# sp-uhh/audio-visual-vad

Measured on NVIDIA B200. Metric: AV-VAD frames/sec (device-timed), higher is better.
Workload: dtype bf16

## Files before the change

### audio-visual-vad_b200/avvad/lib.py

```python
from __future__ import annotations

import ctypes as C
import os
from typing import Optional

_HERE = os.path.dirname(os.path.abspath(__file__))
LIB_PATH = os.path.join(os.path.dirname(_HERE), "lib", "libavvad.so")

c_i32p = C.POINTER(C.c_int32)
c_i64p = C.POINTER(C.c_int64)
c_f32p = C.POINTER(C.c_float)
VP = C.c_void_p

PROTOTYPES = {
    "avvad_last_error": (C.c_char_p, []),
    "avvad_version": (C.c_int, []),
    "avvad_launch_count": (C.c_uint64, []),
    "avvad_profile_enable": (C.c_int, [C.c_int]),
    "avvad_profile_read": (C.c_int, [C.c_int, C.POINTER(C.c_double), C.POINTER(C.c_double), C.POINTER(C.c_uint64)]),
    "avvad_profile_clear": (C.c_int, []),
    "avvad_profile_dump": (C.c_int64, [C.c_int, C.POINTER(C.c_double), C.POINTER(C.c_double), C.c_int64]),
    "avvad_debug_lstm_trace": (None, [VP]),
    "avvad_stft_num_frames": (C.c_int64, [C.c_int64, C.c_double, C.c_double, C.c_double, C.c_int]),
    "avvad_frontend_logpower": (C.c_int, [VP, C.c_int64, VP, VP, C.c_int32, C.c_int32, C.c_int, VP, VP, C.c_float,
                                          VP, VP, VP]),
    "avvad_stft": (C.c_int, [VP, C.c_int64, VP, VP, C.c_int32, C.c_int32, VP, VP]),
    "avvad_upsampled_length": (C.c_int64, [C.c_int64, C.c_int32, C.c_int32]),
    "avvad_upsample_gather": (C.c_int, [VP, C.c_int, VP, VP, C.c_int32, C.c_int32, C.c_int32, C.c_int32, C.c_int32,
                                        C.c_int32, C.c_float, C.c_float, C.c_float, C.c_int, VP, VP]),
    "avvad_upsample_index": (C.c_int, [C.c_int32, C.c_int32, C.c_int32, C.c_int32, VP, VP]),
    "avvad_resnet18_create": (C.c_int, [C.POINTER(VP)]),
    "avvad_resnet18_destroy": (None, [VP]),
    "avvad_resnet18_set_conv": (C.c_int, [VP, C.c_int, VP, VP, VP, VP, VP, C.c_float, VP]),
    "avvad_resnet18_workspace_bytes": (C.c_size_t, [C.c_int64, C.c_int64]),
    "avvad_resnet18_forward": (C.c_int, [VP, VP, C.c_int64, C.c_int64, VP, C.c_size_t, VP, VP, C.c_int64, C.c_int64,
                                         VP]),
    "avvad_resnet18_forward_u8": (C.c_int, [VP, VP, VP, VP, C.c_int32, C.c_int32, C.c_int32, C.c_int32, C.c_int32,
                                            C.c_float, C.c_float, C.c_float, C.c_int, C.c_int64, VP, C.c_size_t, VP, VP,
                                            C.c_int64, C.c_int64, VP]),
    "avvad_resnet18_forward_upto": (C.c_int, [VP, VP, C.c_int64, C.c_int, VP, C.c_size_t, VP, VP]),
    "avvad_resnet18_set_conv_train": (C.c_int, [VP, C.c_int, VP, VP, VP, VP]),
    "avvad_resnet18_train_workspace_bytes": (C.c_size_t, [C.c_int64]),
    "avvad_resnet18_forward_train": (C.c_int, [VP, VP, C.c_int64, VP, C.c_size_t, C.c_float, C.c_float, VP, VP, VP, VP,
                                               C.c_int64, C.c_int64, VP]),
    "avvad_resnet18_tape_bytes": (C.c_size_t, [C.c_int64]),
    "avvad_resnet18_tape_workspace_bytes": (C.c_size_t, [C.c_int64]),
    "avvad_resnet18_tape_layout": (C.c_int, [C.c_int64, c_i64p, C.c_int]),
    "avvad_resnet18_forward_tape": (C.c_int, [VP, VP, C.c_int64, VP, C.c_size_t, VP, C.c_size_t, C.c_float, C.c_float, VP,
                                              VP, VP, VP, C.c_int64, C.c_int64, VP]),
    "avvad_resnet18_backward_workspace_bytes": (C.c_size_t, [C.c_int64]),
    "avvad_resnet18_backward": (C.c_int, [VP, VP, C.c_int64, VP, VP, VP, C.c_size_t, C.c_float, VP, VP, VP, VP]),
    "avvad_gemm_bf16": (C.c_int, [VP, C.c_int64, VP, C.c_int64, VP, VP, C.c_int64, C.c_int, C.c_int, C.c_int64,
                                  C.c_int64, C.c_int64, VP]),
    "avvad_conv2d_nhwc_bf16": (C.c_int, [VP, VP, VP, VP, VP, C.c_int64, C.c_int, C.c_int, C.c_int, C.c_int, C.c_int,
                                         C.c_int, C.c_int, C.c_int, C.c_int, VP]),
    "avvad_dct_roi_workspace_bytes": (C.c_size_t, [C.c_int64]),
    "avvad_dct_roi_decode": (C.c_int, [VP, C.c_int64, C.c_int, VP, VP, VP, C.c_size_t, VP]),
    "avvad_vad_labels": (C.c_int, [VP, C.c_int64, VP, VP, C.c_int32, C.c_int32, C.c_int32, C.c_int32, C.c_double, VP, VP,
                                   VP]),
    "avvad_ibm_labels": (C.c_int, [VP, VP, C.c_int32, C.c_int32, C.c_int32, C.c_float, C.c_float, VP, VP, VP, VP]),
    "avvad_stats_accumulate": (C.c_int, [VP, VP, C.c_int32, C.c_int32, C.c_int32, VP, VP, VP]),
    "avvad_stats_finalize": (C.c_int, [VP, VP, C.c_double, C.c_int32, VP, VP, VP]),
    "avvad_feature_gather": (C.c_int, [VP, VP, VP, VP, C.c_int32, C.c_int32, C.c_int32, C.c_int32, C.c_int32, C.c_int32,
                                       VP, VP, C.c_int64, C.c_int64, VP]),
    "avvad_conv2d_nhwc_bf16_dual": (C.c_int, [VP, VP, VP, VP, VP, C.c_int64] + [C.c_int] * 13 + [VP]),
    "avvad_pack_rows_bf16": (C.c_int, [VP, C.c_int64, VP, C.c_int64, C.c_int64, C.c_int64, C.c_int64, C.c_int, VP]),
    "avvad_mcb_create": (C.c_int, [C.POINTER(VP)]),
    "avvad_mcb_destroy": (None, [VP]),
    "avvad_mcb_load": (C.c_int, [VP, VP, VP, VP, VP, VP, VP, VP, VP, C.c_float, VP]),
    "avvad_mcb_workspace_bytes": (C.c_size_t, [C.c_int64]),
    "avvad_mcb_forward": (C.c_int, [VP, VP, VP, C.c_int64, VP, C.c_size_t, VP, C.c_int64, VP, VP]),
    "avvad_mcb_grouped_workspace_bytes": (C.c_size_t, [C.c_int64, C.c_int64]),
# ... 84 lines not shown
```

### audio-visual-vad_b200/csrc/resnet.cu

```cuda
#include <stdlib.h>

#include <mutex>

#include "gemm_tma.cuh"
#include "stem_s2d.cuh"

namespace avvad {
namespace tc {
int launch_block17(const __nv_bfloat16* x, const __nv_bfloat16* wa, const float* bias_a, const __nv_bfloat16* wb,
                   const float* bias_b, __nv_bfloat16* z, int64_t n, cudaStream_t st);
bool block17_enabled();
}
}

namespace avvad {

struct ConvSpec {
  int cin, cout, k, stride, pad, hin, hout;
};
static const ConvSpec kSpecs[20] = {
    {3, 64, 7, 2, 3, 67, 34},
    {64, 64, 3, 1, 1, 17, 17},   {64, 64, 3, 1, 1, 17, 17},
    {64, 64, 3, 1, 1, 17, 17},   {64, 64, 3, 1, 1, 17, 17},
    {64, 128, 3, 2, 1, 17, 9},   {128, 128, 3, 1, 1, 9, 9},  {64, 128, 1, 2, 0, 17, 9},
// ... 349 lines not shown
  if (chunk <= 0) chunk = 2048;
  return n_frames < chunk ? n_frames : chunk;
}

extern "C" size_t avvad_resnet18_workspace_bytes(int64_t n_frames, int64_t chunk_frames) {
  if (n_frames <= 0) return 0;
  const int64_t mc = chunk_of(n_frames, chunk_frames);
  return (size_t)(4 * align_up((size_t)mc * kActBytesPerFrame, 1024));
}

static int run_conv(avvad_resnet18* h, int layer, const __nv_bfloat16* in, const __nv_bfloat16* residual,
                    __nv_bfloat16* out, int64_t n, int relu, cudaStream_t st) {
  const ConvSpec& s = kSpecs[layer];
  return avvad_conv2d_nhwc_bf16(in, h->w[layer], h->bias[layer], residual, out, n, s.hin, s.hin, s.cin, s.cout, s.k,
                                s.k, s.stride, s.pad, relu, st);
}

struct StemInput {
  const float* frames = nullptr;
  const uint8_t* src = nullptr;
  const int32_t* n_src = nullptr;
  const int32_t* n_out = nullptr;
  int f_max = 0, t_max = 0, num = 0, den = 0, standardise = 0;
  int64_t src_bytes = 0;
  float mean = 0.f, denom = 1.f;
  StemInput advance(int64_t f0) const {
    StemInput r = *this;
    r.first = first + f0;
    return r;
  }
  int64_t first = 0;
};

static int launch_stem_s2d(avvad_resnet18* h, const StemInput& in, int64_t n, __nv_bfloat16* out, cudaStream_t st,
                           const __nv_bfloat16* w = nullptr, const float* bias = nullptr, double* stats = nullptr) {
  static PerDeviceOnce once;
  AVVAD_CUDA(once.run([] {
    cudaError_t e = cudaFuncSetAttribute(tc::stem_s2d_kernel<0>, cudaFuncAttributeMaxDynamicSharedMemorySize, (int)tc::kS2Smem);
    if (e == cudaSuccess)
      e = cudaFuncSetAttribute(tc::stem_s2d_kernel<1>, cudaFuncAttributeMaxDynamicSharedMemorySize, (int)tc::kS2Smem);
    if (e == cudaSuccess)
      e = cudaFuncSetAttribute(tc::stem_s2d_kernel<0, true>, cudaFuncAttributeMaxDynamicSharedMemorySize, (int)tc::kS2Smem);
    return e;
  }));
  static int num_sms = [] {
    int dev = 0, v = 148;
    if (cudaGetDevice(&dev) == cudaSuccess) cudaDeviceGetAttribute(&v, cudaDevAttrMultiProcessorCount, dev);
    return v > 0 ? v : 148;
  }();
  tc::StemS2Params p{};
  p.n_frames = n;
  p.w1b = w ? w : h->w1b;
  p.bias = w ? bias : h->bias[0];
  p.out = out;
  p.stats = stats;
  const int64_t batches = (n + tc::kS2FramesPerBatch - 1) / tc::kS2FramesPerBatch;
  const unsigned grid = (unsigned)(batches < num_sms ? batches : num_sms);
  void* tok = nullptr;
  tc::prof_begin(st, &tok);
  if (in.src) {
    p.src = in.src; p.n_src = in.n_src; p.n_out = in.n_out; p.src_bytes = in.src_bytes;
    p.f_max = in.f_max; p.t_max = in.t_max; p.num = in.num; p.den = in.den;
    p.mean = in.mean; p.denom = in.denom; p.standardise = in.standardise;
    p.first = in.first;
    tc::stem_s2d_kernel<1><<<grid, tc::kS2Threads, tc::kS2Smem, st>>>(p);
  } else if (stats) {
    p.frames = in.frames + in.first * kFrameHW;
    tc::stem_s2d_kernel<0, true><<<grid, tc::kS2Threads, tc::kS2Smem, st>>>(p);
  } else {
    p.frames = in.frames + in.first * kFrameHW;
    tc::stem_s2d_kernel<0><<<grid, tc::kS2Threads, tc::kS2Smem, st>>>(p);
  }
  AVVAD_LAUNCHED();
  tc::prof_end(st, tok, 3, 2.0 * (double)n * 1156 * 64 * 49);
  return AVVAD_OK;
}

static int launch_stem(avvad_resnet18* h, const StemInput& in, int64_t n, __nv_bfloat16* out, cudaStream_t st) {
  return launch_stem_s2d(h, in, n, out, st);
}

static const int64_t kStageIn[4] = {17 * 17 * 64, 17 * 17 * 64, 9 * 9 * 128, 5 * 5 * 256};
static const int64_t kStageOut[4] = {17 * 17 * 64, 9 * 9 * 128, 5 * 5 * 256, 3 * 3 * 512};
static const double kStageMac[4] = {42614784.0, 42467328.0, 52428800.0, 75497472.0};

static int run_trunk_chunk(avvad_resnet18* h, const StemInput& in, int64_t n, __nv_bfloat16* const buf[4], int upto,
                           int* last, cudaStream_t st) {
  if (fuse_ds()) {
    int frc = build_fused(h, st);
    if (frc) return frc;
  }
  const bool whole = upto < 20;
  int cur = 0;
  *last = cur;
  int layer = 1;
  for (int stage = 0; stage < 4; ++stage) {
    {
      const int64_t f0 = 0, nn = n;
// ... 102 lines not shown
        buf[last], n, 9, 512, feat ? feat + f0 * 512 : nullptr,
        feat_bf16 ? (__nv_bfloat16*)feat_bf16 + f0 * ld_bf16 : nullptr, ld_bf16, col_off);
    AVVAD_LAUNCHED();
  }
  return AVVAD_OK;
}

extern "C" int avvad_resnet18_forward(avvad_resnet18* h, const float* frames, int64_t n_frames, int64_t chunk_frames,
                                      void* workspace, size_t workspace_bytes, float* feat, void* feat_bf16,
                                      int64_t ld_bf16, int64_t col_off, void* stream) {
  AVVAD_CHECK_ARG(h && frames && workspace && n_frames > 0, "bad argument");
  StemInput in;
  in.frames = frames;
  return forward_common(h, in, n_frames, chunk_frames, workspace, workspace_bytes, feat, feat_bf16, ld_bf16, col_off,
                        (cudaStream_t)stream);
}

extern "C" int avvad_resnet18_forward_u8(avvad_resnet18* h, const uint8_t* src, const int32_t* n_src,
                                         const int32_t* n_out, int32_t B, int32_t f_max, int32_t t_max, int32_t num,
                                         int32_t den, float mean, float stdv, float eps, int standardise,
                                         int64_t chunk_frames, void* workspace, size_t workspace_bytes, float* feat,
                                         void* feat_bf16, int64_t ld_bf16, int64_t col_off, void* stream) {
  AVVAD_CHECK_ARG(h && src && n_src && n_out && workspace, "null pointer");
  AVVAD_CHECK_ARG(B > 0 && f_max > 0 && t_max > 0 && num > 0 && den > 0, "non-positive size");
  StemInput in;
  in.src = src; in.n_src = n_src; in.n_out = n_out;
  in.f_max = f_max; in.t_max = t_max; in.num = num; in.den = den;
  in.mean = mean; in.denom = stdv + eps; in.standardise = standardise;
  in.src_bytes = (int64_t)B * f_max * kFrameHW;
  return forward_common(h, in, (int64_t)B * t_max, chunk_frames, workspace, workspace_bytes, feat, feat_bf16, ld_bf16,
                        col_off, (cudaStream_t)stream);
}

extern "C" int avvad_resnet18_forward_upto(avvad_resnet18* h, const float* frames, int64_t n_frames, int upto,
                                           void* workspace, size_t workspace_bytes, void* out_act, void* stream) {
  AVVAD_CHECK_ARG(h && frames && workspace && out_act && n_frames > 0 && upto >= 0 && upto < 20, "bad argument");
  int rc = check_loaded(h);
  if (rc) return rc;
  if (workspace_bytes < avvad_resnet18_workspace_bytes(n_frames, n_frames)) {
    set_error("resnet18: workspace too small (forward_upto runs a single chunk)");
    return AVVAD_ERR_WORKSPACE;
  }
  cudaStream_t st = (cudaStream_t)stream;
  const size_t bsz = align_up((size_t)n_frames * kActBytesPerFrame, 1024);
  __nv_bfloat16* buf[4];
  for (int i = 0; i < 4; ++i) buf[i] = reinterpret_cast<__nv_bfloat16*>((uint8_t*)workspace + i * bsz);
  int last = 0;
  StemInput in;
  in.frames = frames;
  rc = run_trunk_chunk(h, in, n_frames, buf, upto, &last, st);
  if (rc) return rc;
  const ConvSpec& s = kSpecs[upto];
  const int ho = (upto == 0) ? 17 : s.hout;
  const size_t bytes = (size_t)n_frames * ho * ho * s.cout * sizeof(__nv_bfloat16);
  AVVAD_CUDA(cudaMemcpyAsync(out_act, buf[last], bytes, cudaMemcpyDeviceToDevice, st));
  return AVVAD_OK;
}

extern "C" int avvad_resnet18_set_conv_train(avvad_resnet18* h, int layer, const float* w, const float* gamma,
                                             const float* beta, void* stream) {
  AVVAD_CHECK_ARG(h && layer >= 0 && layer < 20 && w && gamma && beta, "bad argument");
  cudaStream_t st = (cudaStream_t)stream;
  const ConvSpec& s = kSpecs[layer];
  const size_t wn = (layer == 0) ? 64 * 64 : (size_t)s.cout * s.cin * s.k * s.k;
  if (!h->wraw[layer]) {
    AVVAD_CUDA(cudaMalloc(&h->wraw[layer], wn * sizeof(__nv_bfloat16)));
// ... 142 lines not shown
```

### audio-visual-vad_b200/csrc/stem_s2d.cuh

```cuda
#pragma once
#include "gemm_tc.cuh"

namespace avvad {
namespace tc {

constexpr int kS2Builders = 256;
constexpr int kS2BuilderWarps = kS2Builders / 32;
constexpr int kS2EpiWarps = 8;
constexpr int kS2EpiThreads = kS2EpiWarps * 32;
constexpr int kS2ChPerWarp = 64 / (kS2EpiWarps / 4);
constexpr int kS2Passes = kS2ChPerWarp / 16;
constexpr int kS2Items = (67 * 37 + kS2Builders - 1) / kS2Builders;
constexpr int kS2Threads = kS2Builders + 32 + kS2EpiThreads;
constexpr int kS2FramesPerBatch = 2;
constexpr int kS2RowsPerFrame = 37;
constexpr int kS2Pitch = 160;
constexpr int kS2PlaneRows = 83;
constexpr uint32_t kS2PlaneBytes = kS2PlaneRows * kS2Pitch;
constexpr int kS2EdgeRows = 132;
constexpr uint32_t kS2EdgeChunkBytes = kS2EdgeRows * 16;
constexpr uint32_t kS2EdgePlaneBytes = 2 * kS2EdgeChunkBytes;
constexpr uint32_t kS2BufBytes = 2 * kS2PlaneBytes + 2 * kS2EdgePlaneBytes;
constexpr uint32_t kS2WStepBytes = 256 * 32;
constexpr uint32_t kS2WBytes = 8 * kS2WStepBytes;
constexpr uint32_t kS2OnesBytes = 128 * 32;
constexpr int kS2RingRows = 32;
constexpr uint32_t kS2RingRowBytes = 16 * 128;
constexpr uint32_t kS2RingBytes = kS2RingRows * kS2RingRowBytes;
constexpr uint32_t kS2EdgeHpBytes = 80 * 128;
constexpr uint32_t kS2OffW = 2 * kS2BufBytes;
constexpr uint32_t kS2OffOnes = kS2OffW + kS2WBytes;
constexpr uint32_t kS2OffRing = kS2OffOnes + kS2OnesBytes;
constexpr uint32_t kS2OffEdgeHp = kS2OffRing + kS2RingBytes;
constexpr uint32_t kS2OffLut = kS2OffEdgeHp + kS2EdgeHpBytes;
constexpr uint32_t kS2OffBias = kS2OffLut + 512;
constexpr uint32_t kS2OffBar = kS2OffBias + 256;
constexpr uint32_t kS2StageBytes = 288 * 16;
constexpr uint32_t kS2OffStage = kS2OffBar + 128;
constexpr uint32_t kS2Smem = 1024 + kS2OffStage + 2 * kS2StageBytes;
static_assert(kS2Smem <= 227 * 1024, "stem kernel: shared memory");

struct StemS2Params {
  const float* frames;
  const uint8_t* src;
  const int32_t* n_src;
  const int32_t* n_out;
  int f_max, t_max, num, den;
  float mean, denom;
  int standardise;
  int64_t n_frames;
  int64_t first;
  const __nv_bfloat16* w1b;
  int64_t src_bytes;
  const float* bias;
  __nv_bfloat16* out;
  double* stats;
};

__device__ __forceinline__ uint32_t desc_lo_ns(uint32_t saddr, uint32_t lbo_bytes) {
  return ((saddr & 0x3FFFFu) >> 4) | ((lbo_bytes >> 4) << 16);
}
__device__ __forceinline__ uint32_t desc_hi_ns(uint32_t sbo_bytes) { return (sbo_bytes >> 4) | (1u << 14); }

__device__ __forceinline__ void umma_f16_ns(uint32_t tmem_d, uint32_t a_lo, uint32_t a_hi, uint32_t b_lo, uint32_t b_hi,
                                            uint32_t idesc, uint32_t accum) {
  asm volatile(
      "{\n\t.reg .pred p;\n\t.reg .b64 da, db;\n\t"
      "mov.b64 da, {%1, %2};\n\t"
      "mov.b64 db, {%3, %4};\n\t"
      "setp.ne.b32 p, %6, 0;\n\t"
      "tcgen05.mma.cta_group::1.kind::f16 [%0], da, db, %5, p;\n\t}"
      ::"r"(tmem_d), "r"(a_lo), "r"(a_hi), "r"(b_lo), "r"(b_hi), "r"(idesc), "r"(accum)
      : "memory");
}

__device__ __forceinline__ int s2_src_index(int k, int n_src, int num, int den) {
  long long v = ((long long)den * (2LL * k + 1) - 1) / (2LL * num);
  return v < n_src - 1 ? (int)v : n_src - 1;
}

__device__ __forceinline__ void named_bar_sync(int id, int nthreads) {
  asm volatile("bar.sync %0, %1;" ::"r"(id), "r"(nthreads) : "memory");
}

__device__ __forceinline__ uint32_t bf16x2_max(uint32_t a, uint32_t b) {
  uint32_t r;
  asm("max.bf16x2 %0, %1, %2;" : "=r"(r) : "r"(a), "r"(b));
  return r;
}

template <int MODE, bool STATS = false>
__global__ void __launch_bounds__(kS2Threads, 1) stem_s2d_kernel(const StemS2Params p) {
  extern __shared__ uint8_t smem_raw[];
  const uint32_t raw = smem_u32(smem_raw);
  const uint32_t base = (raw + 1023u) & ~1023u;
  uint8_t* smem = smem_raw + (base - raw);
  float* bias_s = reinterpret_cast<float*>(smem + kS2OffBias);
  unsigned short* lut = reinterpret_cast<unsigned short*>(smem + kS2OffLut);
  const uint32_t bar0 = base + kS2OffBar;
  auto BAR = [&](int i) { return bar0 + 8u * (uint32_t)i; };
  volatile uint32_t* tmem_slot = reinterpret_cast<volatile uint32_t*>(smem + kS2OffBar + 96);

  const int tid = threadIdx.x;
  const int warp = tid >> 5, lane = tid & 31;
  const int64_t n_batches = (p.n_frames + kS2FramesPerBatch - 1) / kS2FramesPerBatch;

  for (uint32_t i = tid; i < (2 * kS2BufBytes) / 16; i += kS2Threads)
    reinterpret_cast<uint4*>(smem)[i] = make_uint4(0u, 0u, 0u, 0u);
  for (int idx = tid; idx < 7 * 256 * 16; idx += kS2Threads) {
    const int e = idx & 15, n = (idx >> 4) & 255, fr = idx >> 12;
    const int s = n >> 6, ch = n & 63;
    const int fs = e - 2 * s;
    __nv_bfloat16 v = __float2bfloat16_rn(0.f);
    if (fs >= 0 && fs < 7) v = p.w1b[ch * 64 + fr * 7 + fs];
    const uint32_t off = kS2OffW + (uint32_t)fr * kS2WStepBytes + (uint32_t)(n >> 3) * 256u + (uint32_t)(e >> 3) * 128u +
                         (uint32_t)(n & 7) * 16u + (uint32_t)(e & 7) * 2u;
    *reinterpret_cast<__nv_bfloat16*>(smem + off) = v;
  }
  for (int idx = tid; idx < 256 * 16; idx += kS2Threads) {
    const int e = idx & 15, n = idx >> 4;
    const float bv = p.bias ? p.bias[n & 63] : 0.f;
    const __nv_bfloat16 hi = __float2bfloat16_rn(bv);
    __nv_bfloat16 v = __float2bfloat16_rn(0.f);
    if (e == 0) v = hi;
    if (e == 1) v = __float2bfloat16_rn(bv - __bfloat162float(hi));
    const uint32_t off = kS2OffW + 7u * kS2WStepBytes + (uint32_t)(n >> 3) * 256u + (uint32_t)(e >> 3) * 128u +
                         (uint32_t)(n & 7) * 16u + (uint32_t)(e & 7) * 2u;
    *reinterpret_cast<__nv_bfloat16*>(smem + off) = v;
  }
  for (uint32_t i = tid; i < kS2OnesBytes / 4; i += kS2Threads)
    reinterpret_cast<uint32_t*>(smem + kS2OffOnes)[i] = 0x3F803F80u;
  if (tid < 64) bias_s[tid] = p.bias ? p.bias[tid] : 0.f;
  if (MODE == 1 && tid < 256) {
    float v = (float)tid;
    if (p.standardise) v = (v - p.mean) / p.denom;
    const __nv_bfloat16 h = __float2bfloat16_rn(v);
    lut[tid] = *reinterpret_cast<const unsigned short*>(&h);
  }
// ... 101 lines not shown
    fetch((int64_t)blockIdx.x * kS2FramesPerBatch);
    for (int64_t bi = blockIdx.x; bi < n_batches; bi += gridDim.x, ++it) {
      const uint32_t buf = it & 1u;
      mbar_wait(BAR(2 + buf), ((it >> 1) & 1u) ^ 1u);
      uint8_t* bufp = smem + buf * kS2BufBytes;
#pragma unroll
      for (int fi = 0; fi < kS2FramesPerBatch; ++fi) {
        const int64_t n = bi * kS2FramesPerBatch + fi;
        const bool have = n < p.n_frames;
        if (have) store();
        if (MODE == 0 && have) build(bufp, fi);
        const int64_t nn = (fi + 1 < kS2FramesPerBatch) ? n + 1 : (bi + gridDim.x) * kS2FramesPerBatch;
        if (fi + 1 < kS2FramesPerBatch || bi + gridDim.x < n_batches) fetch(nn);
        if (MODE == 1 && have) {
          named_bar_sync(2, kS2Builders);
          build(bufp, fi);
        }
      }
      fence_proxy_async();
      mbar_arrive(BAR(0 + buf));
    }
  } else if (warp == kS2BuilderWarps) {
    constexpr uint32_t idesc = make_idesc(256);
    const uint32_t a_hi_main = desc_hi_ns(kS2Pitch), a_hi_edge = desc_hi_ns(128), b_hi = desc_hi_ns(256);
    uint32_t it = 0, g = 0;
    for (int64_t bi = blockIdx.x; bi < n_batches; bi += gridDim.x, ++it) {
      const uint32_t buf = it & 1u;
      const int nf = (int)((p.n_frames - bi * kS2FramesPerBatch) < kS2FramesPerBatch
                               ? (p.n_frames - bi * kS2FramesPerBatch)
                               : kS2FramesPerBatch);
      const int n_main = (nf * kS2RowsPerFrame + 15) / 16;
      mbar_wait(BAR(0 + buf), (it >> 1) & 1u);
      tc_fence_after();
      const uint32_t bufa = base + buf * kS2BufBytes;
      for (int t = -1; t < n_main; ++t, ++g) {
        const uint32_t acc = g & 1u;
        mbar_wait(BAR(6 + acc), ((g >> 1) & 1u) ^ 1u);
        tc_fence_after();
        if (elect_one_sync()) {
          const uint32_t d = tmem_acc + acc * 256u;
          umma_f16_ns(d, desc_lo_ns(base + kS2OffOnes, 128u), b_hi, desc_lo_ns(base + kS2OffW + 7u * kS2WStepBytes, 128u),
                      b_hi, idesc, 0);
#pragma unroll
          for (int fr = 0; fr < 7; ++fr) {
            const int a = fr >> 1, b = fr & 1;
            uint32_t a_lo, a_hi;
            if (t < 0) {
              a_lo = desc_lo_ns(bufa + 2 * kS2PlaneBytes + (uint32_t)b * kS2EdgePlaneBytes + (uint32_t)a * 16u,
                                kS2EdgeChunkBytes);
              a_hi = a_hi_edge;
            } else {
              a_lo = desc_lo_ns(bufa + (uint32_t)b * kS2PlaneBytes + (uint32_t)(16 * t + a) * kS2Pitch, 16u);
              a_hi = a_hi_main;
            }
            const uint32_t b_lo = desc_lo_ns(base + kS2OffW + (uint32_t)fr * kS2WStepBytes, 128u);
            umma_f16_ns(d, a_lo, a_hi, b_lo, b_hi, idesc, 1);
          }
          umma_commit(BAR(4 + acc));
          if (t == n_main - 1) umma_commit(BAR(2 + buf));
        }
        __syncwarp();
      }
    }
  } else {
    const int ew = warp - (kS2BuilderWarps + 1);
    const int q = warp & 3;
    const int half = ew >> 2;
    const int etid = tid - (kS2Builders + 32);
    const int L = q * 32 + lane;
    uint8_t* ring = smem + kS2OffRing;
    uint8_t* edge_hp = smem + kS2OffEdgeHp;
    uint32_t g = 0;
    if (STATS) {
      float sa[kS2ChPerWarp], sq[kS2ChPerWarp];
#pragma unroll
      for (int c = 0; c < kS2ChPerWarp; ++c) sa[c] = sq[c] = 0.f;
      for (int64_t bi = blockIdx.x; bi < n_batches; bi += gridDim.x) {
        const int nf = (int)((p.n_frames - bi * kS2FramesPerBatch) < kS2FramesPerBatch
                                 ? (p.n_frames - bi * kS2FramesPerBatch)
                                 : kS2FramesPerBatch);
        const int n_rows = nf * kS2RowsPerFrame;
        const int n_main = (n_rows + 15) / 16;
        for (int t = -1; t < n_main; ++t, ++g) {
          const uint32_t acc = g & 1u;
          mbar_wait(BAR(4 + acc), (g >> 1) & 1u);
          tc_fence_after();
          const uint32_t t_row = tmem_acc + acc * 256u + ((uint32_t)(q * 32) << 16);
          const int yy = (t < 0) ? L : 16 * t + (L >> 3);
          const int y = yy % kS2RowsPerFrame;
          const bool live = (yy < n_rows) && (y < 34) && (t >= 0 || L < 80);
          const int s_first = (t < 0) ? 2 : 0;
#pragma unroll 1
          for (int pass = 0; pass < kS2Passes; ++pass) {
            const int ch0 = half * kS2ChPerWarp + pass * 16;
#pragma unroll
            for (int sft = 0; sft < 4; ++sft) {
              uint32_t v[16];
              tmem_ld16(t_row + (uint32_t)sft * 64u + ch0, v);
              tmem_ld_wait();
              if (live && sft >= s_first) {
#pragma unroll
                for (int c = 0; c < 16; ++c) {
                  const float x = __uint_as_float(v[c]);
                  if (kS2Passes == 1 || pass == 0) {
                    sa[c] += x;
// ... 5 lines not shown
                }
              }
            }
          }
          tc_fence_before();
          __syncwarp();
          if (lane == 0) mbar_arrive(BAR(6 + acc));
        }
      }
#pragma unroll
      for (int c = 0; c < kS2ChPerWarp; ++c) {
        float a = sa[c], b = sq[c];
#pragma unroll
        for (int o = 16; o > 0; o >>= 1) {
          a += __shfl_xor_sync(0xffffffffu, a, o);
          b += __shfl_xor_sync(0xffffffffu, b, o);
        }
        if (lane == 0) {
          atomicAdd(p.stats + half * kS2ChPerWarp + c, (double)a);
          atomicAdd(p.stats + 64 + half * kS2ChPerWarp + c, (double)b);
        }
      }
    } else
    for (int64_t bi = blockIdx.x; bi < n_batches; bi += gridDim.x) {
      const int nf = (int)((p.n_frames - bi * kS2FramesPerBatch) < kS2FramesPerBatch
                               ? (p.n_frames - bi * kS2FramesPerBatch)
                               : kS2FramesPerBatch);
      const int n_rows = nf * kS2RowsPerFrame;
      const int n_main = (n_rows + 15) / 16;
      for (int t = -1; t < n_main; ++t, ++g) {
        const uint32_t acc = g & 1u;
        mbar_wait(BAR(4 + acc), (g >> 1) & 1u);
        tc_fence_after();
        const uint32_t t_row = tmem_acc + acc * 256u + ((uint32_t)(q * 32) << 16);
        if (t < 0) {
#pragma unroll 1
          for (int pass = 0; pass < kS2Passes; ++pass) {
            const int ch0 = half * kS2ChPerWarp + pass * 16;
            uint32_t v1[16], v2[16], v3[16];
            tmem_ld16(t_row + 64u + ch0, v1);
            tmem_ld16(t_row + 128u + ch0, v2);
            tmem_ld16(t_row + 192u + ch0, v3);
            tmem_ld_wait();
            if (L < 80) {
              uint32_t o[8];
#pragma unroll
              for (int c = 0; c < 8; ++c) {
                const float x0 = fmaxf(fmaxf(__uint_as_float(v1[2 * c]), __uint_as_float(v2[2 * c])), __uint_as_float(v3[2 * c]));
                const float x1 = fmaxf(fmaxf(__uint_as_float(v1[2 * c + 1]), __uint_as_float(v2[2 * c + 1])),
                                       __uint_as_float(v3[2 * c + 1]));
                o[c] = pack_relu_bf16x2(x0, x1);
              }
              uint8_t* rowp = edge_hp + L * 128;
              const int k0 = ch0 >> 3;
              *reinterpret_cast<uint4*>(rowp + (((k0) ^ (L & 7)) << 4)) = make_uint4(o[0], o[1], o[2], o[3]);
              *reinterpret_cast<uint4*>(rowp + (((k0 + 1) ^ (L & 7)) << 4)) = make_uint4(o[4], o[5], o[6], o[7]);
            }
          }
          tc_fence_before();
          __syncwarp();
          if (lane == 0) mbar_arrive(BAR(6 + acc));
          named_bar_sync(1, kS2EpiThreads);
          continue;
        }
        const int yy = 16 * t + (L >> 3);
        const int i = L & 7;
        uint8_t* rrow = ring + (uint32_t)(yy & (kS2RingRows - 1)) * kS2RingRowBytes;
#pragma unroll 1
        for (int pass = 0; pass < kS2Passes; ++pass) {
          const int ch0 = half * kS2ChPerWarp + pass * 16;
          uint32_t v0[16], v1[16], v2[16], v3[16];
          tmem_ld16(t_row + ch0, v0);
          tmem_ld16(t_row + 64u + ch0, v1);
          tmem_ld16(t_row + 128u + ch0, v2);
          tmem_ld16(t_row + 192u + ch0, v3);
          tmem_ld_wait();
          uint32_t oa[8], ob[8];
#pragma unroll
          for (int c = 0; c < 16; c += 2) {
            float pa[2], pb[2];
#pragma unroll
            for (int h = 0; h < 2; ++h) {
              const float s0 = __uint_as_float(v0[c + h]), s1 = __uint_as_float(v1[c + h]);
              const float s2 = __uint_as_float(v2[c + h]), s3 = __uint_as_float(v3[c + h]);
              float left = __shfl_up_sync(0xffffffffu, s3, 1);
              left = (i == 0) ? s0 : left;
              pa[h] = fmaxf(fmaxf(left, s0), s1);
              pb[h] = fmaxf(fmaxf(s1, s2), s3);
            }
            oa[c >> 1] = pack_relu_bf16x2(pa[0], pa[1]);
            ob[c >> 1] = pack_relu_bf16x2(pb[0], pb[1]);
          }
          if (yy < n_rows) {
            const int k0 = ch0 >> 3;
            uint8_t* pxa = rrow + (2 * i) * 128;
            uint8_t* pxb = pxa + 128;
            *reinterpret_cast<uint4*>(pxa + (((k0) ^ i) << 4)) = make_uint4(oa[0], oa[1], oa[2], oa[3]);
            *reinterpret_cast<uint4*>(pxa + (((k0 + 1) ^ i) << 4)) = make_uint4(oa[4], oa[5], oa[6], oa[7]);
            *reinterpret_cast<uint4*>(pxb + (((k0) ^ i) << 4)) = make_uint4(ob[0], ob[1], ob[2], ob[3]);
            *reinterpret_cast<uint4*>(pxb + (((k0 + 1) ^ i) << 4)) = make_uint4(ob[4], ob[5], ob[6], ob[7]);
          }
        }
        tc_fence_before();
        __syncwarp();
        if (lane == 0) mbar_arrive(BAR(6 + acc));
        named_bar_sync(1, kS2EpiThreads);

        {
          const int ch = etid & 7, rr = (etid >> 3) & 7, pg = etid >> 6;
          int ys = 16 * t + 2 * rr;
          int fi = (ys >= kS2RowsPerFrame) ? 1 : 0;
          int y = ys - fi * kS2RowsPerFrame;
          if ((y & 1) == 0) {
            ++ys; ++y;
            if (y == kS2RowsPerFrame) { y = 0; ++fi; }
          }
          if ((y & 1) && y <= 33 && ys < n_rows && fi < nf) {
            const int ph = y >> 1;
            const uint8_t* r0 = ring + (uint32_t)(ys & (kS2RingRows - 1)) * kS2RingRowBytes;
            const uint8_t* r1 = ring + (uint32_t)((ys - 1) & (kS2RingRows - 1)) * kS2RingRowBytes;
            const uint8_t* r2 = ring + (uint32_t)((ys - 2) & (kS2RingRows - 1)) * kS2RingRowBytes;
            const bool top = (y >= 2);
            __nv_bfloat16* orow = p.out + ((bi * kS2FramesPerBatch + fi) * 17 + ph) * (17 * 64) + ch * 8;
#pragma unroll
            for (int pw = pg; pw < 17; pw += kS2EpiThreads / 64) {
              uint4 a, b, c;
              if (pw < 16) {
                const uint32_t off = (uint32_t)pw * 128u + (uint32_t)((ch ^ (pw >> 1)) << 4);
                a = *reinterpret_cast<const uint4*>(r0 + off);
                b = *reinterpret_cast<const uint4*>(r1 + off);
                c = top ? *reinterpret_cast<const uint4*>(r2 + off) : b;
              } else {
                a = *reinterpret_cast<const uint4*>(edge_hp + ys * 128 + ((ch ^ (ys & 7)) << 4));
                b = *reinterpret_cast<const uint4*>(edge_hp + (ys - 1) * 128 + ((ch ^ ((ys - 1) & 7)) << 4));
                c = top ? *reinterpret_cast<const uint4*>(edge_hp + (ys - 2) * 128 + ((ch ^ ((ys - 2) & 7)) << 4)) : b;
              }
              uint4 m;
              m.x = bf16x2_max(bf16x2_max(a.x, b.x), c.x);
              m.y = bf16x2_max(bf16x2_max(a.y, b.y), c.y);
              m.z = bf16x2_max(bf16x2_max(a.z, b.z), c.z);
              m.w = bf16x2_max(bf16x2_max(a.w, b.w), c.w);
              *reinterpret_cast<uint4*>(orow + pw * 64) = m;
            }
          }
        }
        named_bar_sync(1, kS2EpiThreads);
      }
    }
  }

  tc_fence_before();
  __syncthreads();
  if (warp == kS2BuilderWarps) {
    __syncwarp();
    tmem_dealloc(tmem_acc, 512);
  }
}

}
}
```

### include/avvad.h

```cpp
#ifndef AVVAD_H_
#define AVVAD_H_

#include <stddef.h>
#include <stdint.h>

#ifdef __cplusplus
extern "C" {
#endif

typedef enum {
  AVVAD_OK = 0,
  AVVAD_ERR_ARG = -1,
  AVVAD_ERR_CUDA = -2,
  AVVAD_ERR_STATE = -3,
  AVVAD_ERR_WORKSPACE = -4
} avvad_status;

const char* avvad_last_error(void);
int avvad_version(void);
uint64_t avvad_launch_count(void);

int avvad_profile_enable(int on);
int avvad_profile_read(int cat, double* ms, double* flops, uint64_t* launches);
int avvad_profile_clear(void);
int64_t avvad_profile_dump(int cat, double* ms, double* flops, int64_t max_n);
void avvad_debug_lstm_trace(void* buf);


int64_t avvad_stft_num_frames(int64_t n_samples, double fs, double wlen_sec, double hop_percent,
                              int pad_at_end);

int avvad_frontend_logpower(const float* wave, int64_t wave_stride, const int32_t* n_samples,
                            const int32_t* n_frames, int32_t B, int32_t t_max, int normalise,
                            const float* mean, const float* std, float eps, float* out,
                            float* peak_scratch, void* stream);

int avvad_stft(const float* wave, int64_t wave_stride, const int32_t* n_samples,
               const int32_t* n_frames, int32_t B, int32_t t_max, float* out_ft2, void* stream);

int64_t avvad_upsampled_length(int64_t n_src, int32_t num, int32_t den);

int avvad_upsample_gather(const void* src, int src_is_f32, const int32_t* n_src, const int32_t* n_out,
                          int32_t B, int32_t f_max, int32_t t_max, int32_t hw, int32_t num, int32_t den,
                          float mean, float std, float eps, int standardise, float* out, void* stream);

int avvad_feature_gather(const float* feat_src, const float* feat_pad, const int32_t* n_src, const int32_t* n_out,
                         int32_t B, int32_t f_max, int32_t t_max, int32_t C, int32_t num, int32_t den,
                         float* out_f32, void* out_bf16, int64_t ld_bf16, int64_t col_off, void* stream);

int avvad_upsample_index(int32_t n_src, int32_t n_out, int32_t num, int32_t den, int32_t* out_idx,
                         void* stream);

typedef struct avvad_resnet18 avvad_resnet18;

int avvad_resnet18_create(avvad_resnet18** out);
void avvad_resnet18_destroy(avvad_resnet18* h);

int avvad_resnet18_set_conv(avvad_resnet18* h, int layer, const float* w, const float* gamma,
                            const float* beta, const float* mean, const float* var, float bn_eps,
                            void* stream);

size_t avvad_resnet18_workspace_bytes(int64_t n_frames, int64_t chunk_frames);

int avvad_resnet18_forward(avvad_resnet18* h, const float* frames, int64_t n_frames,
                           int64_t chunk_frames, void* workspace, size_t workspace_bytes,
                           float* feat, void* feat_bf16, int64_t ld_bf16, int64_t col_off,
                           void* stream);

int avvad_resnet18_forward_u8(avvad_resnet18* h, const uint8_t* src, const int32_t* n_src,
                              const int32_t* n_out, int32_t B, int32_t f_max, int32_t t_max, int32_t num,
                              int32_t den, float mean, float std, float eps, int standardise,
                              int64_t chunk_frames, void* workspace, size_t workspace_bytes, float* feat,
                              void* feat_bf16, int64_t ld_bf16, int64_t col_off, void* stream);

int avvad_resnet18_forward_upto(avvad_resnet18* h, const float* frames, int64_t n_frames, int upto,
                                void* workspace, size_t workspace_bytes, void* out_act, void* stream);

int avvad_resnet18_set_conv_train(avvad_resnet18* h, int layer, const float* w, const float* gamma, const float* beta,
                                  void* stream);
size_t avvad_resnet18_train_workspace_bytes(int64_t n_frames);
int avvad_resnet18_forward_train(avvad_resnet18* h, const float* frames, int64_t n_frames, void* workspace,
                                 size_t workspace_bytes, float bn_eps, float momentum, float* const* running_mean,
                                 float* const* running_var, float* feat, void* feat_bf16, int64_t ld_bf16,
                                 int64_t col_off, void* stream);

size_t avvad_resnet18_tape_bytes(int64_t n_frames);
size_t avvad_resnet18_tape_workspace_bytes(int64_t n_frames);
int avvad_resnet18_tape_layout(int64_t n_frames, int64_t* offsets, int count);
int avvad_resnet18_forward_tape(avvad_resnet18* h, const float* frames, int64_t n_frames, void* workspace,
                                size_t workspace_bytes, void* tape, size_t tape_bytes, float bn_eps, float momentum,
                                float* const* running_mean, float* const* running_var, float* feat, void* feat_bf16,
                                int64_t ld_bf16, int64_t col_off, void* stream);
size_t avvad_resnet18_backward_workspace_bytes(int64_t n_frames);
int avvad_resnet18_backward(avvad_resnet18* h, const float* frames, int64_t n_frames, void* tape, const float* dfeat,
                            void* workspace, size_t workspace_bytes, float bn_eps, float* const* dW,
                            float* const* dgamma, float* const* dbeta, void* stream);

size_t avvad_dct_roi_workspace_bytes(int64_t n_frames);
int avvad_dct_roi_decode(const float* dct, int64_t n_frames, int mode, uint8_t* out_u8, float* out_f32,
                         void* workspace, size_t workspace_bytes, void* stream);
int avvad_vad_labels(const float* wave, int64_t wave_stride, const int32_t* n_samples, const int32_t* n_frames,
                     int32_t B, int32_t t_max, int32_t nfft, int32_t hop, double vad_threshold,
                     float* energy_scratch, float* labels, void* stream);
int avvad_ibm_labels(const float* stft_ft2, const int32_t* n_frames, int32_t B, int32_t t_max, int32_t bins,
                     float eps, float ibm_threshold, float* db_scratch, float* max_scratch, float* mask,
                     void* stream);
// ... 102 lines not shown
```

Before: 2.131 million.

## Software-pipeline stem epilogue TMEM loads and drop per-tile epilogue barrier

```diff
diff --git a/audio-visual-vad_b200/avvad/lib.py b/audio-visual-vad_b200/avvad/lib.py
--- a/audio-visual-vad_b200/avvad/lib.py
+++ b/audio-visual-vad_b200/avvad/lib.py
@@ -21,6 +21,7 @@
     "avvad_profile_clear": (C.c_int, []),
     "avvad_profile_dump": (C.c_int64, [C.c_int, C.POINTER(C.c_double), C.POINTER(C.c_double), C.c_int64]),
     "avvad_debug_lstm_trace": (None, [VP]),
+    "avvad_debug_stem_trace": (None, [VP]),
     "avvad_stft_num_frames": (C.c_int64, [C.c_int64, C.c_double, C.c_double, C.c_double, C.c_int]),
     "avvad_frontend_logpower": (C.c_int, [VP, C.c_int64, VP, VP, C.c_int32, C.c_int32, C.c_int, VP, VP, C.c_float,
                                           VP, VP, VP]),
@@ -38,6 +39,8 @@
     "avvad_resnet18_forward_u8": (C.c_int, [VP, VP, VP, VP, C.c_int32, C.c_int32, C.c_int32, C.c_int32, C.c_int32,
                                             C.c_float, C.c_float, C.c_float, C.c_int, C.c_int64, VP, C.c_size_t, VP, VP,
                                             C.c_int64, C.c_int64, VP]),
+    "avvad_resnet18_stem_u8": (C.c_int, [VP, VP, VP, VP, C.c_int32, C.c_int32, C.c_int32, C.c_int32, C.c_int32,
+                                         C.c_float, C.c_float, C.c_float, C.c_int, VP, VP]),
     "avvad_resnet18_forward_upto": (C.c_int, [VP, VP, C.c_int64, C.c_int, VP, C.c_size_t, VP, VP]),
     "avvad_resnet18_set_conv_train": (C.c_int, [VP, C.c_int, VP, VP, VP, VP]),
     "avvad_resnet18_train_workspace_bytes": (C.c_size_t, [C.c_int64]),
diff --git a/audio-visual-vad_b200/csrc/resnet.cu b/audio-visual-vad_b200/csrc/resnet.cu
--- a/audio-visual-vad_b200/csrc/resnet.cu
+++ b/audio-visual-vad_b200/csrc/resnet.cu
@@ -405,6 +405,9 @@
   int64_t first = 0;
 };
 
+static unsigned long long* g_stem_trace = nullptr;
+extern "C" void avvad_debug_stem_trace(void* buf) { g_stem_trace = (unsigned long long*)buf; }
+
 static int launch_stem_s2d(avvad_resnet18* h, const StemInput& in, int64_t n, __nv_bfloat16* out, cudaStream_t st,
                            const __nv_bfloat16* w = nullptr, const float* bias = nullptr, double* stats = nullptr) {
   static PerDeviceOnce once;
@@ -412,6 +415,9 @@
     cudaError_t e = cudaFuncSetAttribute(tc::stem_s2d_kernel<0>, cudaFuncAttributeMaxDynamicSharedMemorySize, (int)tc::kS2Smem);
     if (e == cudaSuccess)
       e = cudaFuncSetAttribute(tc::stem_s2d_kernel<1>, cudaFuncAttributeMaxDynamicSharedMemorySize, (int)tc::kS2Smem);
+    if (e == cudaSuccess)
+      e = cudaFuncSetAttribute(tc::stem_s2d_kernel<1, false, true>, cudaFuncAttributeMaxDynamicSharedMemorySize,
+                               (int)tc::kS2Smem);
     if (e == cudaSuccess)
       e = cudaFuncSetAttribute(tc::stem_s2d_kernel<0, true>, cudaFuncAttributeMaxDynamicSharedMemorySize, (int)tc::kS2Smem);
     return e;
@@ -427,6 +433,7 @@
   p.bias = w ? bias : h->bias[0];
   p.out = out;
   p.stats = stats;
+  p.trace = g_stem_trace;
   const int64_t batches = (n + tc::kS2FramesPerBatch - 1) / tc::kS2FramesPerBatch;
   const unsigned grid = (unsigned)(batches < num_sms ? batches : num_sms);
   void* tok = nullptr;
@@ -436,7 +443,10 @@
     p.f_max = in.f_max; p.t_max = in.t_max; p.num = in.num; p.den = in.den;
     p.mean = in.mean; p.denom = in.denom; p.standardise = in.standardise;
     p.first = in.first;
-    tc::stem_s2d_kernel<1><<<grid, tc::kS2Threads, tc::kS2Smem, st>>>(p);
+    if (p.trace)
+      tc::stem_s2d_kernel<1, false, true><<<grid, tc::kS2Threads, tc::kS2Smem, st>>>(p);
+    else
+      tc::stem_s2d_kernel<1><<<grid, tc::kS2Threads, tc::kS2Smem, st>>>(p);
   } else if (stats) {
     p.frames = in.frames + in.first * kFrameHW;
     tc::stem_s2d_kernel<0, true><<<grid, tc::kS2Threads, tc::kS2Smem, st>>>(p);
@@ -605,6 +615,24 @@
                         col_off, (cudaStream_t)stream);
 }
 
+extern "C" int avvad_resnet18_stem_u8(avvad_resnet18* h, const uint8_t* src, const int32_t* n_src,
+                                      const int32_t* n_out, int32_t B, int32_t f_max, int32_t t_max, int32_t num,
+                                      int32_t den, float mean, float stdv, float eps, int standardise, void* out,
+                                      void* stream) {
+  AVVAD_CHECK_ARG(h && src && n_src && n_out && out, "null pointer");
+  AVVAD_CHECK_ARG(B > 0 && f_max > 0 && t_max > 0 && num > 0 && den > 0, "non-positive size");
+  if (!h->set[0]) {
+    set_error("resnet18: conv layer 0 not loaded");
+    return AVVAD_ERR_STATE;
+  }
+  StemInput in;
+  in.src = src; in.n_src = n_src; in.n_out = n_out;
+  in.f_max = f_max; in.t_max = t_max; in.num = num; in.den = den;
+  in.mean = mean; in.denom = stdv + eps; in.standardise = standardise;
+  in.src_bytes = (int64_t)B * f_max * kFrameHW;
+  return launch_stem_s2d(h, in, (int64_t)B * t_max, (__nv_bfloat16*)out, (cudaStream_t)stream);
+}
+
 extern "C" int avvad_resnet18_forward_upto(avvad_resnet18* h, const float* frames, int64_t n_frames, int upto,
                                            void* workspace, size_t workspace_bytes, void* out_act, void* stream) {
   AVVAD_CHECK_ARG(h && frames && workspace && out_act && n_frames > 0 && upto >= 0 && upto < 20, "bad argument");
diff --git a/audio-visual-vad_b200/csrc/stem_s2d.cuh b/audio-visual-vad_b200/csrc/stem_s2d.cuh
--- a/audio-visual-vad_b200/csrc/stem_s2d.cuh
+++ b/audio-visual-vad_b200/csrc/stem_s2d.cuh
@@ -24,7 +24,7 @@
 constexpr uint32_t kS2WStepBytes = 256 * 32;
 constexpr uint32_t kS2WBytes = 8 * kS2WStepBytes;
 constexpr uint32_t kS2OnesBytes = 128 * 32;
-constexpr int kS2RingRows = 32;
+constexpr int kS2RingRows = 34;
 constexpr uint32_t kS2RingRowBytes = 16 * 128;
 constexpr uint32_t kS2RingBytes = kS2RingRows * kS2RingRowBytes;
 constexpr uint32_t kS2EdgeHpBytes = 80 * 128;
@@ -39,6 +39,9 @@
 constexpr uint32_t kS2OffStage = kS2OffBar + 128;
 constexpr uint32_t kS2Smem = 1024 + kS2OffStage + 2 * kS2StageBytes;
 static_assert(kS2Smem <= 227 * 1024, "stem kernel: shared memory");
+constexpr int kS2TraceCtas = 4;
+constexpr int kS2TraceTiles = 2048;
+constexpr int kS2TraceSlots = 8;
 
 struct StemS2Params {
   const float* frames;
@@ -55,6 +58,7 @@
   const float* bias;
   __nv_bfloat16* out;
   double* stats;
+  unsigned long long* trace;
 };
 
 __device__ __forceinline__ uint32_t desc_lo_ns(uint32_t saddr, uint32_t lbo_bytes) {
@@ -89,7 +93,26 @@
   return r;
 }
 
-template <int MODE, bool STATS = false>
+__device__ __forceinline__ void tmem_ld8(uint32_t taddr, uint32_t (&v)[8]) {
+  asm volatile("tcgen05.ld.sync.aligned.32x32b.x8.b32 {%0, %1, %2, %3, %4, %5, %6, %7}, [%8];"
+               : "=r"(v[0]), "=r"(v[1]), "=r"(v[2]), "=r"(v[3]), "=r"(v[4]), "=r"(v[5]), "=r"(v[6]), "=r"(v[7])
+               : "r"(taddr)
+               : "memory");
+}
+__device__ __forceinline__ void tmem_regs_ready(uint32_t (&v)[4][8]) {
+#pragma unroll
+  for (int s = 0; s < 4; ++s)
+#pragma unroll
+    for (int c = 0; c < 8; ++c) asm volatile("" : "+r"(v[s][c]));
+}
+
+__device__ __forceinline__ unsigned long long s2_globaltimer() {
+  unsigned long long t;
+  asm volatile("mov.u64 %0, %%globaltimer;" : "=l"(t));
+  return t;
+}
+
+template <int MODE, bool STATS = false, bool TRACE = false>
 __global__ void __launch_bounds__(kS2Threads, 1) stem_s2d_kernel(const StemS2Params p) {
   extern __shared__ uint8_t smem_raw[];
   const uint32_t raw = smem_u32(smem_raw);
@@ -104,6 +127,11 @@
   const int tid = threadIdx.x;
   const int warp = tid >> 5, lane = tid & 31;
   const int64_t n_batches = (p.n_frames + kS2FramesPerBatch - 1) / kS2FramesPerBatch;
+  unsigned long long* trace =
+      (TRACE && blockIdx.x < kS2TraceCtas) ? p.trace + (size_t)blockIdx.x * kS2TraceTiles * kS2TraceSlots : nullptr;
+  auto stamp = [&](uint32_t tile, int slot) {
+    if (TRACE && trace && tile < (uint32_t)kS2TraceTiles) trace[tile * kS2TraceSlots + slot] = s2_globaltimer();
+  };
 
   for (uint32_t i = tid; i < (2 * kS2BufBytes) / 16; i += kS2Threads)
     reinterpret_cast<uint4*>(smem)[i] = make_uint4(0u, 0u, 0u, 0u);
@@ -271,11 +299,14 @@
       const int n_main = (nf * kS2RowsPerFrame + 15) / 16;
       mbar_wait(BAR(0 + buf), (it >> 1) & 1u);
       tc_fence_after();
+      if (lane == 0) stamp(g, 7);
       const uint32_t bufa = base + buf * kS2BufBytes;
       for (int t = -1; t < n_main; ++t, ++g) {
         const uint32_t acc = g & 1u;
+        if (lane == 0) stamp(g, 5);
         mbar_wait(BAR(6 + acc), ((g >> 1) & 1u) ^ 1u);
         tc_fence_after();
+        if (lane == 0) stamp(g, 6);
         if (elect_one_sync()) {
           const uint32_t d = tmem_acc + acc * 256u;
           umma_f16_ns(d, desc_lo_ns(base + kS2OffOnes, 128u), b_hi, desc_lo_ns(base + kS2OffW + 7u * kS2WStepBytes, 128u),
@@ -310,6 +341,7 @@
     uint8_t* ring = smem + kS2OffRing;
     uint8_t* edge_hp = smem + kS2OffEdgeHp;
     uint32_t g = 0;
+    const bool tr = TRACE && ew == 0 && lane == 0;
     if (STATS) {
       float sa[kS2ChPerWarp], sq[kS2ChPerWarp];
 #pragma unroll
@@ -381,6 +413,7 @@
         const uint32_t acc = g & 1u;
         mbar_wait(BAR(4 + acc), (g >> 1) & 1u);
         tc_fence_after();
+        if (tr) stamp(g, 0);
         const uint32_t t_row = tmem_acc + acc * 256u + ((uint32_t)(q * 32) << 16);
         if (t < 0) {
 #pragma unroll 1
@@ -406,32 +439,34 @@
               *reinterpret_cast<uint4*>(rowp + (((k0 + 1) ^ (L & 7)) << 4)) = make_uint4(o[4], o[5], o[6], o[7]);
             }
           }
+          if (tr) stamp(g, 1);
           tc_fence_before();
           __syncwarp();
           if (lane == 0) mbar_arrive(BAR(6 + acc));
+          if (tr) stamp(g, 2);
           named_bar_sync(1, kS2EpiThreads);
+          if (tr) stamp(g, 3);
           continue;
         }
         const int yy = 16 * t + (L >> 3);
         const int i = L & 7;
-        uint8_t* rrow = ring + (uint32_t)(yy & (kS2RingRows - 1)) * kS2RingRowBytes;
-#pragma unroll 1
-        for (int pass = 0; pass < kS2Passes; ++pass) {
-          const int ch0 = half * kS2ChPerWarp + pass * 16;
-          uint32_t v0[16], v1[16], v2[16], v3[16];
-          tmem_ld16(t_row + ch0, v0);
-          tmem_ld16(t_row + 64u + ch0, v1);
-          tmem_ld16(t_row + 128u + ch0, v2);
-          tmem_ld16(t_row + 192u + ch0, v3);
-          tmem_ld_wait();
-          uint32_t oa[8], ob[8];
-#pragma unroll
-          for (int c = 0; c < 16; c += 2) {
+        uint8_t* pxa = ring + (uint32_t)(yy % kS2RingRows) * kS2RingRowBytes + (2 * i) * 128;
+        uint8_t* pxb = pxa + 128;
+        const bool row_live = yy < n_rows;
+        auto load = [&](uint32_t (&v)[4][8], int pass) {
+          const uint32_t ch0 = (uint32_t)(half * kS2ChPerWarp + pass * 8);
+#pragma unroll
+          for (int sft = 0; sft < 4; ++sft) tmem_ld8(t_row + (uint32_t)sft * 64u + ch0, v[sft]);
+        };
+        auto pool = [&](const uint32_t (&v)[4][8], int pass) {
+          uint32_t oa[4], ob[4];
+#pragma unroll
+          for (int c = 0; c < 8; c += 2) {
             float pa[2], pb[2];
 #pragma unroll
             for (int h = 0; h < 2; ++h) {
-              const float s0 = __uint_as_float(v0[c + h]), s1 = __uint_as_float(v1[c + h]);
-              const float s2 = __uint_as_float(v2[c + h]), s3 = __uint_as_float(v3[c + h]);
+              const float s0 = __uint_as_float(v[0][c + h]), s1 = __uint_as_float(v[1][c + h]);
+              const float s2 = __uint_as_float(v[2][c + h]), s3 = __uint_as_float(v[3][c + h]);
               float left = __shfl_up_sync(0xffffffffu, s3, 1);
               left = (i == 0) ? s0 : left;
               pa[h] = fmaxf(fmaxf(left, s0), s1);
@@ -440,20 +475,37 @@
             oa[c >> 1] = pack_relu_bf16x2(pa[0], pa[1]);
             ob[c >> 1] = pack_relu_bf16x2(pb[0], pb[1]);
           }
-          if (yy < n_rows) {
-            const int k0 = ch0 >> 3;
-            uint8_t* pxa = rrow + (2 * i) * 128;
-            uint8_t* pxb = pxa + 128;
-            *reinterpret_cast<uint4*>(pxa + (((k0) ^ i) << 4)) = make_uint4(oa[0], oa[1], oa[2], oa[3]);
-            *reinterpret_cast<uint4*>(pxa + (((k0 + 1) ^ i) << 4)) = make_uint4(oa[4], oa[5], oa[6], oa[7]);
-            *reinterpret_cast<uint4*>(pxb + (((k0) ^ i) << 4)) = make_uint4(ob[0], ob[1], ob[2], ob[3]);
-            *reinterpret_cast<uint4*>(pxb + (((k0 + 1) ^ i) << 4)) = make_uint4(ob[4], ob[5], ob[6], ob[7]);
-          }
-        }
+          if (row_live) {
+            const int k0 = (half * kS2ChPerWarp + pass * 8) >> 3;
+            *reinterpret_cast<uint4*>(pxa + ((k0 ^ i) << 4)) = make_uint4(oa[0], oa[1], oa[2], oa[3]);
+            *reinterpret_cast<uint4*>(pxb + ((k0 ^ i) << 4)) = make_uint4(ob[0], ob[1], ob[2], ob[3]);
+          }
+        };
+        static_assert(kS2ChPerWarp == 32, "four 8-channel passes per warp");
+        uint32_t va[4][8], vb[4][8];
+        load(va, 0);
+        tmem_ld_wait();
+        tmem_regs_ready(va);
+        load(vb, 1);
+        pool(va, 0);
+        tmem_ld_wait();
+        tmem_regs_ready(vb);
+        load(va, 2);
+        pool(vb, 1);
+        tmem_ld_wait();
+        tmem_regs_ready(va);
+        load(vb, 3);
+        pool(va, 2);
+        tmem_ld_wait();
+        tmem_regs_ready(vb);
+        if (tr) stamp(g, 1);
         tc_fence_before();
         __syncwarp();
         if (lane == 0) mbar_arrive(BAR(6 + acc));
+        pool(vb, 3);
+        if (tr) stamp(g, 2);
         named_bar_sync(1, kS2EpiThreads);
+        if (tr) stamp(g, 3);
 
         {
           const int ch = etid & 7, rr = (etid >> 3) & 7, pg = etid >> 6;
@@ -466,9 +518,11 @@
           }
           if ((y & 1) && y <= 33 && ys < n_rows && fi < nf) {
             const int ph = y >> 1;
-            const uint8_t* r0 = ring + (uint32_t)(ys & (kS2RingRows - 1)) * kS2RingRowBytes;
-            const uint8_t* r1 = ring + (uint32_t)((ys - 1) & (kS2RingRows - 1)) * kS2RingRowBytes;
-            const uint8_t* r2 = ring + (uint32_t)((ys - 2) & (kS2RingRows - 1)) * kS2RingRowBytes;
+            const int s0 = ys % kS2RingRows;
+            const int s1 = s0 ? s0 - 1 : kS2RingRows - 1, s2 = s1 ? s1 - 1 : kS2RingRows - 1;
+            const uint8_t* r0 = ring + (uint32_t)s0 * kS2RingRowBytes;
+            const uint8_t* r1 = ring + (uint32_t)s1 * kS2RingRowBytes;
+            const uint8_t* r2 = ring + (uint32_t)s2 * kS2RingRowBytes;
             const bool top = (y >= 2);
             __nv_bfloat16* orow = p.out + ((bi * kS2FramesPerBatch + fi) * 17 + ph) * (17 * 64) + ch * 8;
 #pragma unroll
@@ -493,7 +547,8 @@
             }
           }
         }
-        named_bar_sync(1, kS2EpiThreads);
+        if (tr) stamp(g, 4);
+        if (t == n_main - 1) named_bar_sync(1, kS2EpiThreads);
       }
     }
   }
diff --git a/include/avvad.h b/include/avvad.h
--- a/include/avvad.h
+++ b/include/avvad.h
@@ -25,6 +25,7 @@
 int avvad_profile_clear(void);
 int64_t avvad_profile_dump(int cat, double* ms, double* flops, int64_t max_n);
 void avvad_debug_lstm_trace(void* buf);
+void avvad_debug_stem_trace(void* buf);
 
 
 int64_t avvad_stft_num_frames(int64_t n_samples, double fs, double wlen_sec, double hop_percent,
@@ -72,6 +73,10 @@
                               int32_t den, float mean, float std, float eps, int standardise,
                               int64_t chunk_frames, void* workspace, size_t workspace_bytes, float* feat,
                               void* feat_bf16, int64_t ld_bf16, int64_t col_off, void* stream);
+
+int avvad_resnet18_stem_u8(avvad_resnet18* h, const uint8_t* src, const int32_t* n_src, const int32_t* n_out,
+                           int32_t B, int32_t f_max, int32_t t_max, int32_t num, int32_t den, float mean, float std,
+                           float eps, int standardise, void* out, void* stream);
 
 int avvad_resnet18_forward_upto(avvad_resnet18* h, const float* frames, int64_t n_frames, int upto,
                                 void* workspace, size_t workspace_bytes, void* out_act, void* stream);
```

New measurement: 2.133 million, median of 6. No clear change (+0.1%).
